# josl/kmerjs

Hardware: AMD Instinct MI355X
Metric: k-mers/sec + distinct-kmers/sec, k=16 150bp synthetic FASTQ, 1/2/4/8 GPU (higher is better)
Workload: dtype u8; 1 GPU; C2: 10000000 synthetic 150bp reads per GPU, k=16, prefix 'ATGAC'; reads_per_gpu=10000000, mode=ordered (reference Map insertion order), k=16, prefix=ATGAC, bytes_per_gpu=3170000000, pipeline=off (steps in sequence), parallelism=dp1 (one GPU; no collective), backend=none

## Files before the change

### kmerjs_amd/csrc/kmer_device.hpp

```cpp
#pragma once
#include "kmer_internal.hpp"

namespace kmerhip {

__device__ __forceinline__ uint32_t wave_incl_sum(uint32_t x) {
    x += (uint32_t)__builtin_amdgcn_update_dpp(0, (int)x, 0x111, 0xf, 0xf, true);
    x += (uint32_t)__builtin_amdgcn_update_dpp(0, (int)x, 0x112, 0xf, 0xf, true);
    x += (uint32_t)__builtin_amdgcn_update_dpp(0, (int)x, 0x114, 0xf, 0xf, true);
    x += (uint32_t)__builtin_amdgcn_update_dpp(0, (int)x, 0x118, 0xf, 0xf, true);
    x += (uint32_t)__builtin_amdgcn_update_dpp(0, (int)x, 0x142, 0xa, 0xf, false);
    x += (uint32_t)__builtin_amdgcn_update_dpp(0, (int)x, 0x143, 0xc, 0xf, false);
    return x;
}

__device__ __forceinline__ uint32_t readlane32(uint32_t v, uint32_t i) {
    return (uint32_t)__builtin_amdgcn_readlane((int)v, (int)i);
}

__device__ __forceinline__ uint64_t readlane64(uint64_t v, uint32_t i) {
    return ((uint64_t)readlane32((uint32_t)(v >> 32), i) << 32) | readlane32((uint32_t)v, i);
}

__device__ __forceinline__ void append_record(Record *recs, unsigned long long *rec_count, uint64_t rec_cap,
                                              unsigned int *err, uint64_t order, uint64_t pos, uint32_t len,
                                              uint32_t strand) {
    const unsigned long long n = atomicAdd(rec_count, 1ull);
    if (n < rec_cap) {
        Record rec;
        rec.order = order;
        rec.pos = pos;
        rec.len = len;
        rec.strand = strand;
        recs[n] = rec;
    } else {
        atomicOr(err, ERR_REC_OVERFLOW);
    }
}

__device__ __forceinline__ uint32_t nl_flags(uint32_t x) {
    uint32_t t = x ^ 0x0A0A0A0Au;
    return ~(t + 0x7F7F7F7Fu) & 0x80808080u;
}

__device__ __forceinline__ uint32_t nl_flags_below(uint32_t x, int64_t n) {
    const uint32_t z = nl_flags(x);
    return n <= 0 ? 0u : n < 4 ? (z & ((1u << (8 * n)) - 1u)) : z;
}

constexpr int NCH_MAIN = TILE / 16;
constexpr int NCH_FRONT = FH / 16;
constexpr int NCH_BACK = BH / 16;
constexpr int BUFSZ = FH + TILE + BH;

__device__ __noinline__ inline uint4 load_chunk_edge(const uint8_t *data, int64_t g, uint64_t len) {
    uint32_t w[4];
#pragma unroll 1
    for (int i = 0; i < 4; ++i) {
        uint32_t x = 0;
        for (int b = 0; b < 4; ++b) {
            const int64_t p = g + i * 4 + b;
            const uint32_t c = (p >= 0 && (uint64_t)p < len) ? data[p] : (uint32_t)'\n';
            x |= c << (8 * b);
        }
        w[i] = x;
    }
    return make_uint4(w[0], w[1], w[2], w[3]);
}

__device__ __forceinline__ uint4 load_chunk(const uint8_t *data, int64_t g, uint64_t len) {
    if (g >= 0 && (uint64_t)g + 16 <= len) return *(const uint4 *)(data + g);
    return load_chunk_edge(data, g, len);
}

struct TileRegs {
    uint4 v[4];
    uint4 vh;
    int hc;
};

__device__ __forceinline__ void load_tile(const uint8_t *data, uint64_t len, int64_t g0, TileRegs &r) {
    const int tid = threadIdx.x;
    const bool halo = tid < NCH_FRONT + NCH_BACK;
    const int hc = tid < NCH_FRONT ? tid : NCH_FRONT + NCH_MAIN + (tid - NCH_FRONT);
    r.hc = hc;
    r.vh = make_uint4(0, 0, 0, 0);
    if (g0 - FH >= 0 && (uint64_t)(g0 + TILE + BH) <= len) {
        const uint8_t *src = data + g0 + 16 * tid;
#pragma unroll
        for (int i = 0; i < 4; ++i) r.v[i] = *(const uint4 *)(src + 16 * TPB * i);
        r.vh = *(const uint4 *)(data + g0 - FH + 16 * (halo ? hc : 0));
    } else {
#pragma unroll
        for (int i = 0; i < 4; ++i) r.v[i] = load_chunk(data, g0 + (int64_t)(tid + TPB * i) * 16, len);
        if (halo) r.vh = load_chunk(data, g0 - FH + (int64_t)hc * 16, len);
    }
}

__device__ __forceinline__ uint32_t store_tile(const TileRegs &r, uint8_t *buf) {
    const int tid = threadIdx.x;
    uint32_t orall = 0;
#pragma unroll
    for (int i = 0; i < 4; ++i) {
        orall |= r.v[i].x | r.v[i].y | r.v[i].z | r.v[i].w;
        *(uint4 *)(buf + FH + (tid + TPB * i) * 16) = r.v[i];
    }
    if (tid < NCH_FRONT + NCH_BACK) *(uint4 *)(buf + r.hc * 16) = r.vh;
    return orall;
}

__device__ __forceinline__ void load_thread_words(const uint8_t *p, uint32_t (&w)[17]) {
    const uint4 *src = (const uint4 *)p;
#pragma unroll
    for (int j = 0; j < 4; ++j) {
        const uint4 x = src[j];
        w[4 * j] = x.x;
        w[4 * j + 1] = x.y;
        w[4 * j + 2] = x.z;
        w[4 * j + 3] = x.w;
    }
    w[16] = *(const uint32_t *)(p + 64);
}

}
```

### kmerjs_amd/csrc/kmer_internal.hpp

```cpp
#pragma once
#include <hip/hip_runtime.h>
#include <stdint.h>

namespace kmerhip {


constexpr int TPB = 256;
constexpr int BPT = 64;
constexpr int TILE = TPB * BPT;
constexpr int FH = 64;
constexpr int BH = 80;
constexpr int KMAX_PACKED = 32;
constexpr int KMAX_TILE = 64;
constexpr int KMAX_DENSE = 32;
constexpr uint32_t MAXREL = (1u << 23) - 1;
constexpr uint32_t PBITS_DEFAULT = 23, PBITS_LONG = 40;
constexpr uint32_t NL_SLOTS = 1024;

enum : uint32_t {
    ERR_NONASCII = 1u << 0,
    ERR_LINE_TOO_LONG = 1u << 1,
    ERR_LOOKBACK_TIMEOUT = 1u << 2,
    ERR_REC_OVERFLOW = 1u << 3,
    ERR_LINE_OVERFLOW = 1u << 4,
    ERR_OVF_OVERFLOW = 1u << 5,
    ERR_CROSS_OVERFLOW = 1u << 6,
    ERR_COUNT_OVERFLOW = 1u << 7,
    ERR_BIG_OVERFLOW = 1u << 8,
    ERR_TAB_SPLIT = 1u << 9,
    ERR_DENSE_RANK = 1u << 10,
    ERR_TAB_CAP = 1u << 11,
    ERR_BKT_CAP = 1u << 12,
    ERR_BKT_RANK = 1u << 13,
    ERR_TAB_LOOKUP = 1u << 14,
    ERR_TAB_EXTRACT = 1u << 15,
    INFO_LONGSEG = 1u << 16,
};
constexpr uint32_t CROSS_HOST_BITS = INFO_LONGSEG | ERR_OVF_OVERFLOW | ERR_REC_OVERFLOW | ERR_CROSS_OVERFLOW;

constexpr uint64_t LB_AGG = 1ull << 62;
constexpr uint64_t LB_INC = 2ull << 62;
constexpr uint64_t LB_VAL = (1ull << 62) - 1;

struct StreamPos {
    uint64_t lines;
    uint64_t unused;
    uint64_t ends_open;
    uint64_t pad;
};

struct Record {
    uint64_t order;
    uint64_t pos;
    uint32_t len;
    uint32_t strand;
};

struct SeqLine {
    uint64_t start;
    uint64_t len;
    uint64_t line_index;
};

struct HitRec {
    uint64_t code;
    uint32_t tile;
    uint32_t qm;
    uint32_t c_local;
    uint32_t lstart;
};
constexpr int HMAX = 64;

struct TileSum {
    uint64_t cnt;
    uint32_t nh;
    uint32_t nx;
    uint64_t lnl;
};

__host__ __device__ inline TileSum tile_sum_op(const TileSum &x, const TileSum &y) {
    TileSum r;
    r.cnt = x.cnt + y.cnt;
    r.nh = x.nh + y.nh;
    r.nx = x.nx + y.nx;
    r.lnl = x.lnl > y.lnl ? x.lnl : y.lnl;
    return r;
}
constexpr uint32_t TSCAN_BLOCK = 1024;
constexpr uint32_t TSCAN_INLINE_MAX = 2048;

struct ScanArgs {
    const uint8_t *data;
    uint64_t len;
    uint64_t abs_offset;
    uint32_t n_tiles, k, plen;
    uint32_t p4, r4, pmask;
    const uint8_t *PR;
    TileSum *tsum;
    HitRec *hits;
    HitRec *ovf;
    unsigned long long *ovf_count;
    uint64_t ovf_cap;
    unsigned int *err;
    uint64_t *hits_hi, *ovf_hi;
};

struct PlaneArgs {
    uint32_t kl[5], kh[5];
    uint32_t rl[5], rh[5];
    uint32_t pb;
};

struct Agg {
    uint64_t first;
    uint64_t count;
};

struct HitArgs {
    const HitRec *hits;
    const TileSum *tsum;
    const TileSum *tscan;
    const HitRec *ovf;
    const unsigned long long *ovf_count;
    uint64_t ovf_cap;
    uint32_t n_tiles, k, plen;
    uint64_t abs_offset;
    const StreamPos *pos;
    uint32_t packed;
    uint32_t pbits;
    uint64_t smask;
    uint64_t invalid_key;
    const uint64_t *hits_hi, *ovf_hi;
    uint32_t wide;
    uint64_t smask_hi;
    uint64_t *rkeyh;
    uint64_t *xkeyh, *xkeyl;
    uint64_t out_base;
    uint64_t rcap;
    uint64_t *rkey;
    uint32_t *rkey32;
    uint64_t *rord;
    uint64_t *xord, *xkey;
    uint32_t *xslot;
    uint64_t xbase, xcap;
    Record *recs;
    unsigned long long *rec_count;
    uint64_t rec_cap;
    unsigned int *err;
    const uint8_t *data;
    uint64_t len;
    uint64_t *scal;
    unsigned int *ticket;
    unsigned long long *chunk_hits, *chunk_cross, *ends_open;
    unsigned int *cross_go;
// ... 690 lines not shown
```

### kmerjs_amd/csrc/kmer_kernels.hip

```cpp
#include "kmer_device.hpp"

#include <algorithm>
#include <cstring>

namespace kmerhip {

__device__ __forceinline__ uint32_t align4(uint32_t hi, uint32_t lo, uint32_t sel) {
    return __builtin_amdgcn_alignbyte(hi, lo, sel);
}

__device__ __forceinline__ void set_info(unsigned int *err, unsigned int bit) {
    if (!(__hip_atomic_load(err, __ATOMIC_RELAXED, __HIP_MEMORY_SCOPE_AGENT) & bit)) atomicOr(err, bit);
}

__device__ __forceinline__ uint32_t not_nl_bits(uint32_t x) {
    return ((x ^ 0x0A0A0A0Au) + 0x7F7F7F7Fu) & 0x80808080u;
}

__device__ __forceinline__ uint32_t not_nl_bits_xad(uint32_t x, uint32_t k0a, uint32_t k7f) {
    uint32_t r;
    asm("v_xad_u32 %0, %1, %2, %3" : "=v"(r) : "v"(x), "v"(k0a), "s"(k7f));
    return r & 0x80808080u;
}

// ... 165 lines not shown
    const uint32_t tile = sh.tile;
    const int64_t g0 = (int64_t)tile * TILE;
    const uint64_t len = a.len;
    uint32_t w[17];
    const uint32_t total = tile_prologue(a.data, len, g0, buf, sh, w, a.err);
    const uint64_t lnl_tile = sh.lastpos >= 0 ? a.abs_offset + (uint64_t)(g0 + sh.lastpos + 1) : 0;

    if (wid == 0) {
        uint64_t lbase, lnlb;
        if (LOOKBACK) {
            if (tile == 0) {
                lbase = a.pos->lines;
                lnlb = a.abs_offset;
                if (lane == 0) {
                    lb_store(a.lb_cnt, LB_INC | (lbase + total));
                    lb_store(a.lb_lnl, LB_INC | (lnl_tile > lnlb ? lnl_tile : lnlb));
                }
            } else {
                if (lane == 0) {
                    lb_store(a.lb_cnt + tile, LB_AGG | total);
                    lb_store(a.lb_lnl + tile, LB_AGG | lnl_tile);
                }
                lbase = look_back<true>(a.lb_cnt, tile, a.err);
                lnlb = look_back<false>(a.lb_lnl, tile, a.err);
                if (lane == 0) {
                    lb_store(a.lb_cnt + tile, LB_INC | (lbase + total));
                    lb_store(a.lb_lnl + tile, LB_INC | (lnl_tile > lnlb ? lnl_tile : lnlb));
                }
            }
            if (tile == a.n_tiles - 1 && lane == 0) {
                a.pos->lines = lbase + total;
                a.pos->ends_open = (len > 0 && a.data[len - 1] != '\n') ? 1 : 0;
            }
        } else {
            lbase = a.tp_cnt[tile];
            lnlb = a.tp_lnl[tile];
        }
        if (lane == 0) {
            sh.line_base = lbase;
            sh.lnl_before = lnlb;
        }
    }
    __syncthreads();
    const uint64_t lbase = sh.line_base;
#pragma unroll 1
    for (int i = 0; i < 64; ++i) {
        const int q = 64 * tid + i;
        if ((uint64_t)(g0 + q) >= len) break;
        if (buf[FH + q - 1] != '\n') continue;
        const uint32_t c = sh.tpre[tid] + nl_before_in_thread(buf, tid, q);
        const uint64_t li = lbase + c;
        if ((li & 3) != 1) continue;
        int64_t e = g0 + q;
        while ((uint64_t)e < len && (e - g0 < TILE + BH ? buf[FH + (e - g0)] : a.data[e]) != '\n') ++e;
        const uint64_t L = (uint64_t)e - (uint64_t)(g0 + q);
        if (L > 1 && L >= a.k) {
            const unsigned long long n = atomicAdd(a.line_count, 1ull);
            if (n < a.line_cap) {
                a.lines_out[n].start = (uint64_t)(g0 + q);
                a.lines_out[n].len = L;
                a.lines_out[n].line_index = li;
            } else {
                atomicOr(a.err, ERR_LINE_OVERFLOW);
            }
        }
    }
}

constexpr int QCAP = 256;

struct alignas(16) ScanShared {
    uint16_t cpre[NCH_MAIN];
    uint32_t nlmap[NCH_MAIN / 32];
    uint32_t wsum[TPB / 64][4];
    int32_t last_chunk;
    int32_t lastpos;
    uint32_t nh;
    uint32_t nx;
    uint32_t tcnt;
    uint32_t qn;
    alignas(8) uint32_t q[QCAP];
};

__device__ __forceinline__ void put_tile_hits(const ScanArgs &a, const ScanShared &sh, uint32_t tile) {
    a.tsum[tile].nh = sh.nh;
    a.tsum[tile].nx = sh.nh > (uint32_t)HMAX ? sh.nh : sh.nx;
    if (sh.nh > (uint32_t)HMAX || (sh.nh && sh.tcnt == 0)) set_info(a.err, INFO_LONGSEG);
}

__device__ __forceinline__ int last_newline_in_chunk(const uint8_t *buf, int c, int limit = 1 << 30) {
    const uint4 x = *(const uint4 *)(buf + FH + 16 * c);
    const uint32_t xs[4] = {x.x, x.y, x.z, x.w};
    int last = -1;
#pragma unroll
    for (int j = 0; j < 4; ++j) {
        const int pos = 16 * c + 4 * j;
        const int rem = limit - pos;
        uint32_t z = nl_flags(xs[j]);
        z = rem <= 0 ? 0u : rem < 4 ? (z & ((1u << (8 * rem)) - 1u)) : z;
        last = z ? pos + ((31 - __clz(z)) >> 3) : last;
    }
    return last;
}

__host__ __device__ constexpr uint32_t byte_range_mask(int from, int to) {
    from = from < 0 ? 0 : from > 4 ? 4 : from;
    to = to < 0 ? 0 : to > 4 ? 4 : to;
    const uint32_t a = to >= 4 ? ~0u : (1u << (8 * to)) - 1u, b = from >= 4 ? ~0u : (1u << (8 * from)) - 1u;
    return a & ~b;
}

__device__ __forceinline__ uint32_t acgt_diff(uint32_t x) {
    const uint32_t c = ((x >> 1) ^ (x >> 2)) & 0x03030303u;
    return __builtin_amdgcn_perm(0u, 0x54474341u, c) ^ x;
}

__device__ __forceinline__ void line_context_chunks(const uint8_t *buf, const ScanShared &sh, int s0,
                                                    uint32_t &c_local, int &lstart) {
    const int cs = (s0 - 1) >> 4;
    const uint4 x4 = *(const uint4 *)(buf + FH + 16 * cs);
    const uint32_t xs[4] = {x4.x, x4.y, x4.z, x4.w};
    uint32_t cnt = 0;
    int last = -1;
#pragma unroll
    for (int j = 0; j < 4; ++j) {
        const int pos = 16 * cs + 4 * j;
        const int rem = s0 - pos;
        uint32_t z = nl_flags(xs[j]);
        z = rem <= 0 ? 0u : rem < 4 ? (z & ((1u << (8 * rem)) - 1u)) : z;
        cnt += __popc(z);
        last = z ? pos + ((31 - __clz(z)) >> 3) : last;
    }
    c_local = (uint32_t)sh.cpre[cs] + cnt;
    if (last >= 0) {
        lstart = last + 1;
    } else if (c_local > 0) {
        const int cc = cs - 1;
        int wi = cc >> 5;
        uint32_t m = sh.nlmap[wi] & (0xFFFFFFFFu >> (31 - (cc & 31)));
        while (m == 0) m = sh.nlmap[--wi];
        lstart = last_newline_in_chunk(buf, 32 * wi + 31 - __clz(m)) + 1;
    }
}

__device__ __forceinline__ uint32_t chunk_nl_mask(uint4 x) {
    const uint32_t k0a = 0x0A0A0A0Au, k7f = 0x7F7F7F7Fu;
    const uint32_t lo = __builtin_amdgcn_udot4(not_nl_bits_xad(x.y, k0a, k7f), 0x80402010u,
                            __builtin_amdgcn_udot4(not_nl_bits_xad(x.x, k0a, k7f), 0x08040201u, 0u, false), false);
    const uint32_t hi = __builtin_amdgcn_udot4(not_nl_bits_xad(x.w, k0a, k7f), 0x80402010u,
                            __builtin_amdgcn_udot4(not_nl_bits_xad(x.z, k0a, k7f), 0x08040201u, 0u, false), false);
    return ~((lo >> 7) | (hi << 1)) & 0xFFFFu;
}

__device__ __forceinline__ void line_context_regions(const uint8_t *buf, const ScanShared &sh, int s0, bool want,
                                                     uint32_t &c_local, int &lstart) {
    const int cs = (s0 > 0 ? s0 - 1 : 0) >> 4;
    const int rg = cs >> 2, wi = rg >> 5;
    const uint4 x4 = *(const uint4 *)(buf + FH + 16 * cs);
    const uint2 c2 = *(const uint2 *)(sh.cpre + 4 * rg);
    const uint32_t mhi = sh.nlmap[wi], mlo = sh.nlmap[wi > 0 ? wi - 1 : 0];
    const uint32_t cnt = __popc(__builtin_amdgcn_ubfe(chunk_nl_mask(x4), 0u, (uint32_t)(s0 - 16 * cs)));
    const uint32_t ccs = (uint32_t)((((uint64_t)c2.y << 32) | c2.x) >> (16 * (cs & 3))) & 0xFFFFu;
    const uint32_t cl = ccs + cnt;
    const bool has = want && cl > 0;
    int R = rg;
    if (has && cnt == 0 && ccs == (c2.x & 0xFFFFu)) {
        const uint64_t m = (((uint64_t)mhi << 32) | (wi > 0 ? mlo : 0u)) & ((1ull << (32 + (rg & 31))) - 1ull);
        R = 32 * (wi - 1) + 63 - (int)__clzll((long long)m);
        if (m == 0) {
            int w = wi - 1;
            uint32_t mm;
            do mm = sh.nlmap[--w]; while (mm == 0);
            R = 32 * w + 31 - __clz(mm);
        }
    }
    const uint2 d2 = *(const uint2 *)(sh.cpre + 4 * R);
    const uint32_t nxt = sh.cpre[min(4 * R + 4, NCH_MAIN - 1)];
    const uint32_t d[4] = {d2.x & 0xFFFFu, d2.x >> 16, d2.y & 0xFFFFu, d2.y >> 16};
    const int jl = R == rg ? cs - 4 * rg : 4;
    const int jc = (jl > 3 && d[3] < nxt) ? 3 : (jl > 2 && d[2] < d[3]) ? 2 : (jl > 1 && d[1] < d[2]) ? 1 : 0;
    const int c = cnt ? cs : 4 * R + jc;
    const uint4 y4 = *(const uint4 *)(buf + FH + 16 * c);
    const uint32_t ym = __builtin_amdgcn_ubfe(chunk_nl_mask(y4), 0u, (uint32_t)min(s0 - 16 * c, 16));
    const int last = 16 * c + 31 - __clz(ym);
    c_local = want ? cl : 0u;
    lstart = has ? last + 1 : -1;
}

template <bool THREAD_MAP, bool WIDE, uint32_t K = 0, uint32_t PLEN = 0>
__device__ __forceinline__ void emit_hit(const ScanArgs &a, const uint8_t *buf, ScanShared &sh, uint32_t tile,
                                         uint32_t e, uint32_t pb = 0, const uint32_t *pw = nullptr) {
    static_assert((K == 0) == (PLEN == 0) && PLEN <= 5 && PLEN <= K && K <= (WIDE ? KMAX_TILE : KMAX_PACKED),
                  "fixed k / prefix length: both or neither, prefix fully plane-tested");
    const uint32_t k = K ? K : a.k, plen = K ? PLEN : a.plen;
    const uint32_t strand = e & 1u;
    const int q = (int)(e >> 1);
    const int s0 = strand ? q + (int)plen - (int)k : q;
    uint32_t exo_bits = 0, nl_bits = 0;
    uint32_t pfx_bits = 0;
    uint64_t code = 0;
    const int sfx0 = strand ? 0 : (int)plen, sfx1 = strand ? (int)(k - plen) : (int)k;
#pragma unroll 4
    for (uint32_t b = 0; b < k; b += 4) {
        const uint32_t x = lds_word(buf, s0 + (int)b);
        const uint32_t nb = k - b >= 4 ? 4u : k - b;
        const uint32_t mk = nb == 4 ? 0xFFFFFFFFu : ((1u << (8 * nb)) - 1u);
        const uint32_t c = ((x >> 1) ^ (x >> 2)) & 0x03030303u;
        const uint32_t expect = __builtin_amdgcn_perm(0u, 0x54474341u, c);
        if (THREAD_MAP && K) {
            const uint32_t pf = byte_range_mask(0 - (int)b, (int)PLEN - (int)b),
                           pr = byte_range_mask((int)K - (int)PLEN - (int)b, (int)K - (int)b);
            const uint32_t pm = strand ? pr : pf;
            pfx_bits |= (expect ^ x) & mk & pm;
            exo_bits |= (expect ^ x) & mk & ~pm;
        } else {
            const uint32_t mx = THREAD_MAP ? mk : mk & byte_range_mask(sfx0 - (int)b, sfx1 - (int)b);
            exo_bits |= (expect ^ x) & mx;
        }
        nl_bits |= nl_flags(x) & mk;
        const uint32_t pk = __builtin_amdgcn_udot4(c, 0x01041040u, 0u, false);
        code = (code << (2 * nb)) | (pk >> (2 * (4 - nb)));
    }
    if (THREAD_MAP && !K) {
        pfx_bits = (acgt_diff(lds_word(buf, q)) & (pb >= 4 ? 0xFFFFFFFFu : ((1u << (8 * pb)) - 1u))) |
                   (acgt_diff(lds_word(buf, q + 4)) & (pb > 4 ? 0xFFu : 0u));
        for (uint32_t b = 4; b < plen && plen > 5; b += 4) {
            const uint32_t n = plen - b;
            const uint32_t mk = (n >= 4 ? 0xFFFFFFFFu : ((1u << (8 * n)) - 1u)) & (b == 4 ? 0xFFFFFF00u : 0xFFFFFFFFu);
            pfx_bits |= (lds_word(buf, q + (int)b) ^ pw[(strand ? KMAX_TILE / 4 : 0) + b / 4]) & mk;
        }
    }
    const bool exotic = exo_bits != 0, hasnl = nl_bits != 0;
    uint64_t chi = 0;
    if (WIDE) {
        for (uint32_t b = 0; b < k - 32; b += 4) {
            const uint32_t x = lds_word(buf, s0 + (int)b);
            const uint32_t nb = k - 32 - b >= 4 ? 4u : k - 32 - b;
            const uint32_t c = ((x >> 1) ^ (x >> 2)) & 0x03030303u;
            const uint32_t pk = __builtin_amdgcn_udot4(c, 0x01041040u, 0u, false);
            chi = (chi << (2 * nb)) | (pk >> (2 * (4 - nb)));
        }
    }
    const bool valid = pfx_bits == 0 && !hasnl &&
                       !(k == 1 && buf[FH + s0 - 1] == '\n' && buf[FH + s0 + 1] == '\n');
    uint32_t c_local = 0;
    int lstart = -1;
    if (THREAD_MAP) line_context_regions(buf, sh, s0, valid && s0 > 0, c_local, lstart);
    else if (valid && s0 > 0) line_context_chunks(buf, sh, s0, c_local, lstart);
    const bool cross = valid && (lstart < 0 || c_local == sh.tcnt);
    const unsigned long long vm = __ballot(valid), xm = __ballot(cross), act = __ballot(1);
    const int lane = threadIdx.x & 63, leader = __ffsll((long long)act) - 1;
    uint32_t base = 0;
    if (lane == leader) {
        if (vm) base = atomicAdd(&sh.nh, (uint32_t)__popcll(vm));
        if (xm) atomicAdd(&sh.nx, (uint32_t)__popcll(xm));
    }
    base = (uint32_t)__shfl((int)base, leader);
    if (!valid) return;
    const uint32_t slot = base + (uint32_t)__popcll(vm & ((1ull << lane) - 1ull));
    HitRec r;
    r.code = code;
    r.tile = tile;
    r.qm = (uint32_t)q | (strand << 14) | ((exotic ? 1u : 0u) << 15) | ((lstart >= 0 ? 1u : 0u) << 16) | (slot << 17);
    r.c_local = c_local;
    r.lstart = lstart >= 0 ? (uint32_t)lstart : 0u;
    if (slot < HMAX) {
        a.hits[(uint64_t)tile * HMAX + slot] = r;
        if (WIDE) a.hits_hi[(uint64_t)tile * HMAX + slot] = chi;
    } else {
        const unsigned long long o = atomicAdd(a.ovf_count, 1ull);
        if (o < a.ovf_cap) {
            a.ovf[o] = r;
            if (WIDE) a.ovf_hi[o] = chi;
        } else {
            atomicOr(a.err, ERR_OVF_OVERFLOW);
        }
    }
}

template <bool WIDE>
__device__ __forceinline__ void scan_word(const ScanArgs &a, const uint8_t *buf, ScanShared &sh, uint32_t tile,
                                          const uint32_t *pw, uint32_t q0) {
    const uint32_t plen = a.plen, P4 = a.p4, R4 = a.r4, PM = a.pmask;
    const uint32_t lo = *(const uint32_t *)(buf + FH + q0);
    const uint32_t hi = *(const uint32_t *)(buf + FH + q0 + 4);
    uint32_t bits = 0;
#pragma unroll
    for (uint32_t jj = 0; jj < 4; ++jj) {
        const uint32_t win = align4(hi, lo, jj);
        bits |= (((win ^ P4) & PM) == 0 ? 1u : 0u) << (2 * jj);
        bits |= (((win ^ R4) & PM) == 0 ? 1u : 0u) << (2 * jj + 1);
    }
    while (bits) {
        const uint32_t bit = __ffs(bits) - 1;
        bits &= bits - 1;
        const uint32_t strand = bit & 1u;
        const int q = (int)q0 + (int)(bit >> 1);
        bool ok = true;
#pragma unroll 1
        for (uint32_t b = 4; b < plen && ok; b += 4) {
            const uint32_t n = plen - b;
            const uint32_t mk = n >= 4 ? 0xFFFFFFFFu : ((1u << (8 * n)) - 1u);
            ok = ((lds_word(buf, q + (int)b) ^ pw[(strand ? KMAX_TILE / 4 : 0) + b / 4]) & mk) == 0;
        }
        if (ok) emit_hit<false, WIDE>(a, buf, sh, tile, ((uint32_t)q << 1) | strand);
    }
}

template <bool FULL4, bool WIDE>
__global__ __launch_bounds__(TPB) void scan_tile_kernel(ScanArgs a) {
    __shared__ __attribute__((aligned(16))) uint8_t buf[BUFSZ];
    __shared__ ScanShared sh;
    __shared__ __attribute__((aligned(16))) uint8_t s_pr[2 * KMAX_TILE];
    const int tid = threadIdx.x, lane = tid & 63, wid = tid >> 6;
    const uint64_t len = a.len;
    const uint32_t tile = blockIdx.x;
    const int64_t g0 = (int64_t)tile * TILE;
    {
        uint8_t prb = 0;
        if (tid < 2 * KMAX_TILE) prb = a.PR[tid];
        TileRegs r;
        load_tile(a.data, len, g0, r);
        if (tid == 0) {
            sh.last_chunk = -1;
            sh.nh = 0;
            sh.nx = 0;
            sh.qn = 0;
        }
        const uint32_t orall = store_tile(r, buf);
        if (tid < 2 * KMAX_TILE) s_pr[tid] = prb;
        if (orall & 0x80808080u) atomicOr(a.err, ERR_NONASCII);
    }
// ... 63 lines not shown
            }
        }
        const uint64_t excl = incl - packed;
        uint32_t base = 0;
#pragma unroll
        for (int i = 0; i < 4; ++i) {
            sh.cpre[tid + TPB * i] = (uint16_t)(base + col_off[i] + ((excl >> (16 * i)) & 0xFFFFu));
            base += col_total[i];
        }
        if (tid == 0) {
            a.tsum[tile].cnt = base;
            sh.tcnt = base;
        }
    }
    if (tid == 0) {
        const int lc = sh.last_chunk;
        const int64_t lim = (int64_t)len - g0;
        const int lp = lc >= 0 ? last_newline_in_chunk(buf, lc, lim < TILE ? (int)lim : TILE) : -1;
        sh.lastpos = lp;
        a.tsum[tile].lnl = lp >= 0 ? a.abs_offset + (uint64_t)(g0 + lp + 1) : 0;
    }
    const uint32_t k = a.k, plen = a.plen;
    if (plen > k) cand = 0;
    const uint32_t *pw = (const uint32_t *)s_pr;

    __syncthreads();
    {
        const uint32_t nc = __popc(cand);
        const uint32_t incl_c = wave_incl_sum(nc);
        const uint32_t wtotal = (uint32_t)__builtin_amdgcn_readlane((int)incl_c, 63);
        uint32_t pos = 0;
        if (wtotal) {
            uint32_t base = 0;
            if (lane == 0) base = atomicAdd(&sh.qn, wtotal);
            pos = (uint32_t)__builtin_amdgcn_readfirstlane((int)__shfl((int)base, 0)) + incl_c - nc;
        }
        while (cand) {
            const int bitc = __ffs(cand) - 1;
            cand &= cand - 1;
            const uint32_t q0 = 16u * (uint32_t)(tid + TPB * (bitc >> 2)) + 4u * (uint32_t)(bitc & 3);
            if (pos < QCAP) sh.q[pos] = q0;
            else scan_word<WIDE>(a, buf, sh, tile, pw, q0);
            ++pos;
        }
    }
    __syncthreads();
    const uint32_t nq = min(sh.qn, (uint32_t)QCAP);
    for (uint32_t h = tid; h < nq; h += TPB) scan_word<WIDE>(a, buf, sh, tile, pw, sh.q[h]);
    if (nq > 64 || sh.qn > QCAP) {
        __syncthreads();
        if (tid == 0) put_tile_hits(a, sh, tile);
    } else if (tid == 0) {
        put_tile_hits(a, sh, tile);
    }
}


__device__ __forceinline__ uint32_t plane_match(uint32_t L0, uint32_t H0, uint32_t L1, uint32_t H1,
                                                const uint32_t *kl, const uint32_t *kh, uint32_t pb,
                                                const uint32_t *SL, const uint32_t *SH) {
    uint32_t acc = (L0 ^ kl[0]) & (H0 ^ kh[0]);
#pragma unroll
    for (uint32_t i = 1; i < 5; ++i) {
        if (i < pb) acc = acc & (SL[i] ^ kl[i]) & (SH[i] ^ kh[i]);
    }
    return acc;
}

__host__ __device__ constexpr uint32_t plane_masks_const(const char *p, const char *r) {
    uint32_t m = 0;
    for (int i = 0; i < 5; ++i) {
        const uint32_t cp = (((uint32_t)p[i] >> 1) & 1u) | ((((uint32_t)p[i] >> 2) & 1u) << 1);
        const uint32_t cr = (((uint32_t)r[i] >> 1) & 1u) | ((((uint32_t)r[i] >> 2) & 1u) << 1);
        m |= ((cp & 1u) ? 0u : 1u) << (4 * i);
        m |= ((cp & 2u) ? 0u : 1u) << (4 * i + 1);
        m |= ((cr & 1u) ? 0u : 1u) << (4 * i + 2);
        m |= ((cr & 2u) ? 0u : 1u) << (4 * i + 3);
    }
    return m;
}
constexpr uint32_t PM_ATGAC = plane_masks_const("ATGAC", "GTCAT");

template <bool FULL5, bool WIDE, uint32_t PM = 0, uint32_t K = 0, uint32_t PLEN = 0>
__global__ __launch_bounds__(TPB) void scan_planes_kernel(ScanArgs a, PlaneArgs pa) {
    __shared__ __attribute__((aligned(16))) uint8_t buf[BUFSZ];
    __shared__ ScanShared sh;
    __shared__ __attribute__((aligned(16))) uint8_t s_pr[2 * KMAX_TILE];
    const int tid = threadIdx.x, lane = tid & 63, wid = tid >> 6;
    const uint64_t len = a.len;
    const uint32_t tile = blockIdx.x;
    const int64_t g0 = (int64_t)tile * TILE;
    {
        uint8_t prb = 0;
        if (K == 0 && tid < 2 * KMAX_TILE) prb = a.PR[tid];
        TileRegs r;
        load_tile(a.data, len, g0, r);
        if (tid == 0) {
            sh.last_chunk = -1;
            sh.nh = 0;
            sh.nx = 0;
            sh.qn = 0;
        }
        const uint32_t orall = store_tile(r, buf);
        if (K == 0 && tid < 2 * KMAX_TILE) s_pr[tid] = prb;
        if (orall & 0x80808080u) atomicOr(a.err, ERR_NONASCII);
    }
    __syncthreads();

    uint32_t w[17];
    load_thread_words(buf + FH + 64 * tid, w);
    const bool tail_tile = (uint64_t)(g0 + TILE) > len;
    const uint32_t k0a = 0x0A0A0A0Au, k7f = 0x7F7F7F7Fu;
    uint32_t ccnt[4];
#pragma unroll
    for (int j = 0; j < 4; ++j) {
        uint32_t cnt = 0;
        if (!tail_tile) {
#pragma unroll
            for (int i = 0; i < 4; ++i) cnt += __popc(not_nl_bits_xad(w[4 * j + i], k0a, k7f));
            cnt = 16u - cnt;
        } else {
            const int64_t gc = g0 + 64 * tid + 16 * j;
#pragma unroll
            for (int i = 0; i < 4; ++i) cnt += __popc(nl_flags_below(w[4 * j + i], (int64_t)len - (gc + 4 * i)));
        }
        ccnt[j] = cnt;
    }
    const uint32_t ttot = ccnt[0] + ccnt[1] + ccnt[2] + ccnt[3];
    {
        const unsigned long long m = __ballot(ttot != 0);
        if (lane == 0) {
            sh.nlmap[2 * wid] = (uint32_t)m;
            sh.nlmap[2 * wid + 1] = (uint32_t)(m >> 32);
            if (m) atomicMax(&sh.last_chunk, 64 * wid + 63 - (int)__clzll((long long)m));
        }
    }
    const uint32_t incl = wave_incl_sum(ttot);
    if (lane == 63) sh.wsum[wid][0] = incl;

    const uint32_t W0 = 0x08040201u;
    uint32_t L[3], H[3];
#pragma unroll
    for (int h = 0; h < 2; ++h) {
        uint32_t gl[4], gh[4];
#pragma unroll
        for (int p = 0; p < 4; ++p) {
            const uint32_t x0 = w[8 * h + 2 * p], x1 = w[8 * h + 2 * p + 1];
            uint32_t y;
            asm("v_bfi_b32 %0, %1, %2, %3" : "=v"(y) : "s"(0x0F0F0F0Fu), "v"(x0), "v"(x1 << 4));
            gl[p] = __builtin_amdgcn_udot4(y & 0x22222222u, W0, 0u, false);
            gh[p] = __builtin_amdgcn_udot4(y & 0x44444444u, W0, 0u, false);
        }
        L[h] = (gl[0] >> 1) | (gl[1] << 7) | (gl[2] << 15) | (gl[3] << 23);
        H[h] = (gh[0] >> 2) | (gh[1] << 6) | (gh[2] << 14) | (gh[3] << 22);
    }
    {
        const uint32_t x = w[16];
        L[2] = __builtin_amdgcn_udot4(x & 0x02020202u, W0, 0u, false) >> 1;
        H[2] = __builtin_amdgcn_udot4(x & 0x04040404u, W0, 0u, false) >> 2;
    }
    uint32_t mf[2], mr[2];
    const uint32_t pb = FULL5 ? 5u : pa.pb;
    uint32_t kl[5], kh[5], rl[5], rh[5];
#pragma unroll
    for (int i = 0; i < 5; ++i) {
        if constexpr (PM != 0) {
            kl[i] = ((PM >> (4 * i)) & 1u) ? ~0u : 0u;
            kh[i] = ((PM >> (4 * i + 1)) & 1u) ? ~0u : 0u;
            rl[i] = ((PM >> (4 * i + 2)) & 1u) ? ~0u : 0u;
            rh[i] = ((PM >> (4 * i + 3)) & 1u) ? ~0u : 0u;
        } else {
            kl[i] = pa.kl[i];
            kh[i] = pa.kh[i];
            rl[i] = pa.rl[i];
            rh[i] = pa.rh[i];
        }
    }
#pragma unroll
    for (int h = 0; h < 2; ++h) {
        uint32_t SL[5], SH[5];
        SL[0] = L[h];
        SH[0] = H[h];
#pragma unroll
        for (uint32_t i = 1; i < 5; ++i) {
            SL[i] = __builtin_amdgcn_alignbit(L[h + 1], L[h], i);
            SH[i] = __builtin_amdgcn_alignbit(H[h + 1], H[h], i);
        }
        mf[h] = plane_match(L[h], H[h], L[h + 1], H[h + 1], kl, kh, pb, SL, SH);
        mr[h] = plane_match(L[h], H[h], L[h + 1], H[h + 1], rl, rh, pb, SL, SH);
    }
    if (!K && a.k < a.plen) mf[0] = mf[1] = mr[0] = mr[1] = 0;

    __syncthreads();
    {
        uint32_t pre = incl - ttot, tot = 0;
#pragma unroll
        for (int ww = 0; ww < TPB / 64; ++ww) {
            pre += ww < wid ? sh.wsum[ww][0] : 0u;
            tot += sh.wsum[ww][0];
        }
#pragma unroll
        for (int j = 0; j < 4; ++j) {
            sh.cpre[4 * tid + j] = (uint16_t)pre;
            pre += ccnt[j];
        }
        if (tid == 0) {
            a.tsum[tile].cnt = tot;
            sh.tcnt = tot;
        }
    }
    __syncthreads();
    if (tid == 0) {
        const int lt = sh.last_chunk;
        int lp = -1;
        if (lt >= 0) {
            int c = 4 * lt + 3;
            while ((c == NCH_MAIN - 1 ? sh.tcnt : (uint32_t)sh.cpre[c + 1]) == sh.cpre[c]) --c;
            const int64_t lim = (int64_t)len - g0;
            lp = last_newline_in_chunk(buf, c, lim < TILE ? (int)lim : TILE);
        }
        sh.lastpos = lp;
        a.tsum[tile].lnl = lp >= 0 ? a.abs_offset + (uint64_t)(g0 + lp + 1) : 0;
    }

    const uint32_t *pw = (const uint32_t *)s_pr;
    uint2 *qe = (uint2 *)sh.q;
    constexpr uint32_t QE = QCAP / 2;
    static_assert(QE == 128 && QCAP == 256, "a round: one entry per thread of waves 0 and 1, 128 queue words each");
    const uint32_t mm[4] = {mf[0], mf[1], mr[0], mr[1]};
    uint32_t qpos[4] = {0, 0, 0, 0};
    {
        unsigned long long bl[4];
        uint32_t tot = 0;
#pragma unroll
        for (int hs = 0; hs < 4; ++hs) {
            bl[hs] = __ballot(mm[hs] != 0);
            tot += (uint32_t)__popcll(bl[hs]);
        }
        if (tot) {
            uint32_t base = 0;
            if (lane == 0) base = atomicAdd(&sh.qn, tot);
            base = (uint32_t)__builtin_amdgcn_readfirstlane((int)base);
#pragma unroll
            for (int hs = 0; hs < 4; ++hs) {
                qpos[hs] = base + __builtin_amdgcn_mbcnt_hi((uint32_t)(bl[hs] >> 32),
                                                            __builtin_amdgcn_mbcnt_lo((uint32_t)bl[hs], 0u));
                base += (uint32_t)__popcll(bl[hs]);
            }
        }
    }
    auto enqueue = [&](uint32_t done) {
#pragma unroll
        for (int hs = 0; hs < 4; ++hs) {
            const uint32_t e0 = ((64u * (uint32_t)tid + 32u * (uint32_t)(hs & 1)) << 1) | (uint32_t)(hs >> 1);
            if (mm[hs] && qpos[hs] - done < QE) qe[qpos[hs] - done] = make_uint2(e0, mm[hs]);
        }
    };
    enqueue(0);
    __syncthreads();
    const uint32_t total = sh.qn;
    if (total <= 64 && wid != 0) return;
    for (uint32_t done = 0;;) {
        const uint32_t left = total - done;
        uint2 en = make_uint2(0u, 0u);
        if ((uint32_t)tid < min(left, QE)) en = qe[tid];
        const uint32_t nc = __popc(en.y), incl = wave_incl_sum(nc);
        const uint32_t wtot = readlane32(incl, 63);
        uint32_t *flat = sh.q + 128 * (wid & 1);
        for (uint32_t cb = 0; cb < wtot; cb += 64) {
            uint32_t m = en.y, p = incl - nc - cb;
            while (m) {
                const uint32_t bit = __ffs(m) - 1;
                m &= m - 1;
                if (p < 64) flat[p] = en.x + (bit << 1);
                ++p;
            }
            if ((uint32_t)lane < min(wtot - cb, 64u))
                emit_hit<true, WIDE, K, PLEN>(a, buf, sh, tile, flat[lane], pb, pw);
        }
        if (left <= QE) break;
        __syncthreads();
        done += QE;
        enqueue(done);
        __syncthreads();
    }
    if (total > 64) __syncthreads();
    if (tid == 0) put_tile_hits(a, sh, tile);
}

__device__ __forceinline__ uint64_t resolve_hit(const HitArgs &a, uint64_t pos_lines, const HitRec &r,
                                                uint64_t code_hi, const TileSum &tb, uint64_t *order_out,
                                                uint32_t *lk, bool *lvalid_out, uint64_t *key_hi) {
    const uint32_t t = r.tile;
    const uint32_t strand = (r.qm >> 14) & 1u;
    const bool exotic = (r.qm >> 15) & 1u;
    const bool lvalid = (r.qm >> 16) & 1u;
    const int q = (int)(r.qm & 0x3FFFu);
    const int s0 = strand ? q + (int)a.plen - (int)a.k : q;
    const uint64_t tile_abs = a.abs_offset + (uint64_t)t * TILE;
    const uint64_t li = pos_lines + tb.cnt + r.c_local;
    const uint64_t lstart = lvalid ? tile_abs + r.lstart : tb.lnl;
    const uint64_t sabs = tile_abs + (uint64_t)(int64_t)s0;
    uint64_t rel = sabs - lstart;
    const bool seq = (li & 3) == 1;
    const uint64_t maxrel = (1ull << a.pbits) - 1ull;
    if (rel > maxrel) {
        if (seq) atomicOr(a.err, ERR_LINE_TOO_LONG);
        rel = maxrel;
    }
    if (li >> (63 - a.pbits)) atomicOr(a.err, ERR_LINE_TOO_LONG);
    const uint64_t order = (li << (a.pbits + 1)) | ((uint64_t)strand << a.pbits) | (strand ? maxrel - rel : rel);
    *order_out = order;
    const uint32_t sp = (uint32_t)(s0 + 64);
    *lk = (r.c_local << 17) | (strand << 16) | (strand ? 0xFFFFu - sp : sp);
    *lvalid_out = lvalid;
    uint64_t key = a.invalid_key;
    *key_hi = a.wide ? a.invalid_key : 0;
    if (a.wide) key = 0;
    if (seq) {
        if (a.packed && !exotic) {
            if (a.k > 32) {
                uint64_t h = code_hi, l = r.code;
                if (strand) revcomp_code128(code_hi, r.code, a.k, &h, &l);
                key = l & a.smask;
                *key_hi = h & a.smask_hi;
            } else {
                key = (strand ? revcomp_code(r.code, a.k) : r.code) & a.smask;
            }
        } else {
            append_record(a.recs, a.rec_count, a.rec_cap, a.err, order, (uint64_t)t * TILE + (uint64_t)(int64_t)s0, a.k,
                          strand);
        }
    }
    return key;
}

__device__ __forceinline__ void place_hit(const HitArgs &a, uint64_t slot, bool cross, uint64_t xi, uint64_t key,
                                          uint64_t key_hi, uint64_t order) {
    if (!cross) {
        if (slot >= a.rcap) {
            atomicOr(a.err, ERR_OVF_OVERFLOW);
            return;
        }
        if (a.rkey32) a.rkey32[slot] = (uint32_t)key;
        else a.rkey[slot] = key;
        if (a.wide) a.rkeyh[slot] = key_hi;
        a.rord[slot] = order;
    } else if (xi < a.xcap) {
        a.xord[xi] = order;
        a.xslot[xi] = (uint32_t)slot;
        if (a.wide) {
            a.xkey[xi] = xi;
            a.xkeyl[xi] = key;
            a.xkeyh[xi] = key_hi;
        } else {
            a.xkey[xi] = key;
        }
    } else {
        atomicOr(a.err, ERR_CROSS_OVERFLOW);
    }
}
// ... 2359 lines not shown
```

Measured before the change: 3487 billion k-mers/s.

## Carry per-hit line context in queue and drop barrier-heavy prefix pass in plane scan

The plane-scan kernel no longer builds a shared per-chunk newline prefix table or runs the serial last-newline search behind two extra block barriers. Each thread computes a 64-bit newline mask, a wave prefix count and a wave max of its last-newline position, and stores this context next to its queued hits. Emitters then derive the line start and local count from that mask with popcount/clz instead of walking shared tables. The change also adds nontemporal loads for the main tile and an 8-waves-per-EU occupancy hint, at the cost of a larger shared struct (a 16-byte context per queue entry) and extra packing logic on the queue entries.

After: 3795 billion k-mers/s (median of 6 runs). 1.09x the previous value.

```diff
diff --git a/kmerjs_amd/csrc/kmer_device.hpp b/kmerjs_amd/csrc/kmer_device.hpp
--- a/kmerjs_amd/csrc/kmer_device.hpp
+++ b/kmerjs_amd/csrc/kmer_device.hpp
@@ -10,6 +10,16 @@
     x += (uint32_t)__builtin_amdgcn_update_dpp(0, (int)x, 0x118, 0xf, 0xf, true);
     x += (uint32_t)__builtin_amdgcn_update_dpp(0, (int)x, 0x142, 0xa, 0xf, false);
     x += (uint32_t)__builtin_amdgcn_update_dpp(0, (int)x, 0x143, 0xc, 0xf, false);
+    return x;
+}
+
+__device__ __forceinline__ uint32_t wave_incl_max(uint32_t x) {
+    x = max(x, (uint32_t)__builtin_amdgcn_update_dpp(0, (int)x, 0x111, 0xf, 0xf, true));
+    x = max(x, (uint32_t)__builtin_amdgcn_update_dpp(0, (int)x, 0x112, 0xf, 0xf, true));
+    x = max(x, (uint32_t)__builtin_amdgcn_update_dpp(0, (int)x, 0x114, 0xf, 0xf, true));
+    x = max(x, (uint32_t)__builtin_amdgcn_update_dpp(0, (int)x, 0x118, 0xf, 0xf, true));
+    x = max(x, (uint32_t)__builtin_amdgcn_update_dpp(0, (int)x, 0x142, 0xa, 0xf, false));
+    x = max(x, (uint32_t)__builtin_amdgcn_update_dpp(0, (int)x, 0x143, 0xc, 0xf, false));
     return x;
 }
 
@@ -78,6 +88,7 @@
     int hc;
 };
 
+template <bool NT = false>
 __device__ __forceinline__ void load_tile(const uint8_t *data, uint64_t len, int64_t g0, TileRegs &r) {
     const int tid = threadIdx.x;
     const bool halo = tid < NCH_FRONT + NCH_BACK;
@@ -87,7 +98,15 @@
     if (g0 - FH >= 0 && (uint64_t)(g0 + TILE + BH) <= len) {
         const uint8_t *src = data + g0 + 16 * tid;
 #pragma unroll
-        for (int i = 0; i < 4; ++i) r.v[i] = *(const uint4 *)(src + 16 * TPB * i);
+        for (int i = 0; i < 4; ++i) {
+            if constexpr (NT) {
+                typedef uint32_t u32x4 __attribute__((ext_vector_type(4)));
+                const u32x4 t = __builtin_nontemporal_load((const u32x4 *)(src + 16 * TPB * i));
+                r.v[i] = make_uint4(t.x, t.y, t.z, t.w);
+            } else {
+                r.v[i] = *(const uint4 *)(src + 16 * TPB * i);
+            }
+        }
         r.vh = *(const uint4 *)(data + g0 - FH + 16 * (halo ? hc : 0));
     } else {
 #pragma unroll
diff --git a/kmerjs_amd/csrc/kmer_internal.hpp b/kmerjs_amd/csrc/kmer_internal.hpp
--- a/kmerjs_amd/csrc/kmer_internal.hpp
+++ b/kmerjs_amd/csrc/kmer_internal.hpp
@@ -70,6 +70,16 @@
     uint32_t lstart;
 };
 constexpr int HMAX = 64;
+
+__host__ __device__ inline void region_line_context(uint32_t pre, int32_t prevnl, uint64_t mask, uint32_t qrel,
+                                                    int32_t base, uint32_t *c_local, int32_t *lstart) {
+    const uint64_t below = mask & ((1ull << qrel) - 1ull);
+    const uint32_t lo = (uint32_t)below, hi = (uint32_t)(below >> 32);
+    *c_local = pre + (uint32_t)__builtin_popcount(lo) + (uint32_t)__builtin_popcount(hi);
+    const int32_t own = hi ? 64 - __builtin_clz(hi) : 32 - __builtin_clz(lo | 1u);
+    const int32_t ls = below ? base + own : prevnl + 1;
+    *lstart = ls > 0 ? ls : -1;
+}
 
 struct TileSum {
     uint64_t cnt;
diff --git a/kmerjs_amd/csrc/kmer_kernels.hip b/kmerjs_amd/csrc/kmer_kernels.hip
--- a/kmerjs_amd/csrc/kmer_kernels.hip
+++ b/kmerjs_amd/csrc/kmer_kernels.hip
@@ -271,7 +271,21 @@
     alignas(8) uint32_t q[QCAP];
 };
 
-__device__ __forceinline__ void put_tile_hits(const ScanArgs &a, const ScanShared &sh, uint32_t tile) {
+constexpr uint32_t QE = QCAP / 2;
+struct alignas(16) PlaneShared {
+    uint32_t wsum[TPB / 64];
+    uint32_t wmax[TPB / 64];
+    uint32_t nh;
+    uint32_t nx;
+    uint32_t tcnt;
+    uint32_t qn;
+    uint2 q[QE];
+    uint4 qc[QE];
+    uint32_t flat[2][64];
+};
+
+template <class SH>
+__device__ __forceinline__ void put_tile_hits(const ScanArgs &a, const SH &sh, uint32_t tile) {
     a.tsum[tile].nh = sh.nh;
     a.tsum[tile].nx = sh.nh > (uint32_t)HMAX ? sh.nh : sh.nx;
     if (sh.nh > (uint32_t)HMAX || (sh.nh && sh.tcnt == 0)) set_info(a.err, INFO_LONGSEG);
@@ -332,53 +346,10 @@
     }
 }
 
-__device__ __forceinline__ uint32_t chunk_nl_mask(uint4 x) {
-    const uint32_t k0a = 0x0A0A0A0Au, k7f = 0x7F7F7F7Fu;
-    const uint32_t lo = __builtin_amdgcn_udot4(not_nl_bits_xad(x.y, k0a, k7f), 0x80402010u,
-                            __builtin_amdgcn_udot4(not_nl_bits_xad(x.x, k0a, k7f), 0x08040201u, 0u, false), false);
-    const uint32_t hi = __builtin_amdgcn_udot4(not_nl_bits_xad(x.w, k0a, k7f), 0x80402010u,
-                            __builtin_amdgcn_udot4(not_nl_bits_xad(x.z, k0a, k7f), 0x08040201u, 0u, false), false);
-    return ~((lo >> 7) | (hi << 1)) & 0xFFFFu;
-}
-
-__device__ __forceinline__ void line_context_regions(const uint8_t *buf, const ScanShared &sh, int s0, bool want,
-                                                     uint32_t &c_local, int &lstart) {
-    const int cs = (s0 > 0 ? s0 - 1 : 0) >> 4;
-    const int rg = cs >> 2, wi = rg >> 5;
-    const uint4 x4 = *(const uint4 *)(buf + FH + 16 * cs);
-    const uint2 c2 = *(const uint2 *)(sh.cpre + 4 * rg);
-    const uint32_t mhi = sh.nlmap[wi], mlo = sh.nlmap[wi > 0 ? wi - 1 : 0];
-    const uint32_t cnt = __popc(__builtin_amdgcn_ubfe(chunk_nl_mask(x4), 0u, (uint32_t)(s0 - 16 * cs)));
-    const uint32_t ccs = (uint32_t)((((uint64_t)c2.y << 32) | c2.x) >> (16 * (cs & 3))) & 0xFFFFu;
-    const uint32_t cl = ccs + cnt;
-    const bool has = want && cl > 0;
-    int R = rg;
-    if (has && cnt == 0 && ccs == (c2.x & 0xFFFFu)) {
-        const uint64_t m = (((uint64_t)mhi << 32) | (wi > 0 ? mlo : 0u)) & ((1ull << (32 + (rg & 31))) - 1ull);
-        R = 32 * (wi - 1) + 63 - (int)__clzll((long long)m);
-        if (m == 0) {
-            int w = wi - 1;
-            uint32_t mm;
-            do mm = sh.nlmap[--w]; while (mm == 0);
-            R = 32 * w + 31 - __clz(mm);
-        }
-    }
-    const uint2 d2 = *(const uint2 *)(sh.cpre + 4 * R);
-    const uint32_t nxt = sh.cpre[min(4 * R + 4, NCH_MAIN - 1)];
-    const uint32_t d[4] = {d2.x & 0xFFFFu, d2.x >> 16, d2.y & 0xFFFFu, d2.y >> 16};
-    const int jl = R == rg ? cs - 4 * rg : 4;
-    const int jc = (jl > 3 && d[3] < nxt) ? 3 : (jl > 2 && d[2] < d[3]) ? 2 : (jl > 1 && d[1] < d[2]) ? 1 : 0;
-    const int c = cnt ? cs : 4 * R + jc;
-    const uint4 y4 = *(const uint4 *)(buf + FH + 16 * c);
-    const uint32_t ym = __builtin_amdgcn_ubfe(chunk_nl_mask(y4), 0u, (uint32_t)min(s0 - 16 * c, 16));
-    const int last = 16 * c + 31 - __clz(ym);
-    c_local = want ? cl : 0u;
-    lstart = has ? last + 1 : -1;
-}
-
-template <bool THREAD_MAP, bool WIDE, uint32_t K = 0, uint32_t PLEN = 0>
-__device__ __forceinline__ void emit_hit(const ScanArgs &a, const uint8_t *buf, ScanShared &sh, uint32_t tile,
-                                         uint32_t e, uint32_t pb = 0, const uint32_t *pw = nullptr) {
+template <bool THREAD_MAP, bool WIDE, uint32_t K = 0, uint32_t PLEN = 0, class SH>
+__device__ __forceinline__ void emit_hit(const ScanArgs &a, const uint8_t *buf, SH &sh, uint32_t tile,
+                                         uint32_t e, uint32_t pb = 0, const uint32_t *pw = nullptr,
+                                         uint4 lc = make_uint4(0u, 0u, 0u, 0u), uint32_t tcnt = 0) {
     static_assert((K == 0) == (PLEN == 0) && PLEN <= 5 && PLEN <= K && K <= (WIDE ? KMAX_TILE : KMAX_PACKED),
                   "fixed k / prefix length: both or neither, prefix fully plane-tested");
     const uint32_t k = K ? K : a.k, plen = K ? PLEN : a.plen;
@@ -434,9 +405,14 @@
                        !(k == 1 && buf[FH + s0 - 1] == '\n' && buf[FH + s0 + 1] == '\n');
     uint32_t c_local = 0;
     int lstart = -1;
-    if (THREAD_MAP) line_context_regions(buf, sh, s0, valid && s0 > 0, c_local, lstart);
-    else if (valid && s0 > 0) line_context_chunks(buf, sh, s0, c_local, lstart);
-    const bool cross = valid && (lstart < 0 || c_local == sh.tcnt);
+    if constexpr (THREAD_MAP) {
+        region_line_context(lc.x, (int)lc.w - 1, ((uint64_t)lc.z << 32) | lc.y, (uint32_t)q & 63u, q & ~63, &c_local,
+                            &lstart);
+    } else {
+        if (valid && s0 > 0) line_context_chunks(buf, sh, s0, c_local, lstart);
+        tcnt = sh.tcnt;
+    }
+    const bool cross = valid && (lstart < 0 || c_local == tcnt);
     const unsigned long long vm = __ballot(valid), xm = __ballot(cross), act = __ballot(1);
     const int lane = threadIdx.x & 63, leader = __ffsll((long long)act) - 1;
     uint32_t base = 0;
@@ -666,9 +642,9 @@
 constexpr uint32_t PM_ATGAC = plane_masks_const("ATGAC", "GTCAT");
 
 template <bool FULL5, bool WIDE, uint32_t PM = 0, uint32_t K = 0, uint32_t PLEN = 0>
-__global__ __launch_bounds__(TPB) void scan_planes_kernel(ScanArgs a, PlaneArgs pa) {
+__global__ __launch_bounds__(TPB) __attribute__((amdgpu_waves_per_eu(8))) void scan_planes_kernel(ScanArgs a, PlaneArgs pa) {
     __shared__ __attribute__((aligned(16))) uint8_t buf[BUFSZ];
-    __shared__ ScanShared sh;
+    __shared__ PlaneShared sh;
     __shared__ __attribute__((aligned(16))) uint8_t s_pr[2 * KMAX_TILE];
     const int tid = threadIdx.x, lane = tid & 63, wid = tid >> 6;
     const uint64_t len = a.len;
@@ -678,9 +654,8 @@
         uint8_t prb = 0;
         if (K == 0 && tid < 2 * KMAX_TILE) prb = a.PR[tid];
         TileRegs r;
-        load_tile(a.data, len, g0, r);
+        load_tile<true>(a.data, len, g0, r);
         if (tid == 0) {
-            sh.last_chunk = -1;
             sh.nh = 0;
             sh.nx = 0;
             sh.qn = 0;
@@ -695,32 +670,32 @@
     load_thread_words(buf + FH + 64 * tid, w);
     const bool tail_tile = (uint64_t)(g0 + TILE) > len;
     const uint32_t k0a = 0x0A0A0A0Au, k7f = 0x7F7F7F7Fu;
-    uint32_t ccnt[4];
-#pragma unroll
-    for (int j = 0; j < 4; ++j) {
-        uint32_t cnt = 0;
-        if (!tail_tile) {
-#pragma unroll
-            for (int i = 0; i < 4; ++i) cnt += __popc(not_nl_bits_xad(w[4 * j + i], k0a, k7f));
-            cnt = 16u - cnt;
-        } else {
-            const int64_t gc = g0 + 64 * tid + 16 * j;
-#pragma unroll
-            for (int i = 0; i < 4; ++i) cnt += __popc(nl_flags_below(w[4 * j + i], (int64_t)len - (gc + 4 * i)));
-        }
-        ccnt[j] = cnt;
-    }
-    const uint32_t ttot = ccnt[0] + ccnt[1] + ccnt[2] + ccnt[3];
-    {
-        const unsigned long long m = __ballot(ttot != 0);
-        if (lane == 0) {
-            sh.nlmap[2 * wid] = (uint32_t)m;
-            sh.nlmap[2 * wid + 1] = (uint32_t)(m >> 32);
-            if (m) atomicMax(&sh.last_chunk, 64 * wid + 63 - (int)__clzll((long long)m));
-        }
-    }
+    uint32_t nm[2];
+#pragma unroll
+    for (int h = 0; h < 2; ++h) {
+        uint32_t d[4];
+#pragma unroll
+        for (int p = 0; p < 4; ++p)
+            d[p] = __builtin_amdgcn_udot4(not_nl_bits_xad(w[8 * h + 2 * p + 1], k0a, k7f), 0x80402010u,
+                       __builtin_amdgcn_udot4(not_nl_bits_xad(w[8 * h + 2 * p], k0a, k7f), 0x08040201u, 0u, false), false);
+        nm[h] = ~((d[0] >> 7) | (d[1] << 1) | (d[2] << 9) | (d[3] << 17));
+    }
+    if (tail_tile) {
+        const int64_t left = (int64_t)len - (g0 + 64 * tid);
+        const uint64_t keep = left >= 64 ? ~0ull : left <= 0 ? 0ull : (1ull << left) - 1ull;
+        nm[0] &= (uint32_t)keep;
+        nm[1] &= (uint32_t)(keep >> 32);
+    }
+    const uint32_t ttot = __popc(nm[0]) + __popc(nm[1]);
+    const uint32_t mylast = nm[1] ? 64u * (uint32_t)tid + 64u - (uint32_t)__clz(nm[1])
+                                  : nm[0] ? 64u * (uint32_t)tid + 32u - (uint32_t)__clz(nm[0]) : 0u;
     const uint32_t incl = wave_incl_sum(ttot);
-    if (lane == 63) sh.wsum[wid][0] = incl;
+    const uint32_t inclmax = wave_incl_max(mylast);
+    if (lane == 63) {
+        sh.wsum[wid] = incl;
+        sh.wmax[wid] = inclmax;
+    }
+    uint32_t prev1 = (uint32_t)__builtin_amdgcn_update_dpp(0, (int)inclmax, 0x138, 0xf, 0xf, true);
 
     const uint32_t W0 = 0x08040201u;
     uint32_t L[3], H[3];
@@ -775,42 +750,10 @@
     }
     if (!K && a.k < a.plen) mf[0] = mf[1] = mr[0] = mr[1] = 0;
 
-    __syncthreads();
-    {
-        uint32_t pre = incl - ttot, tot = 0;
-#pragma unroll
-        for (int ww = 0; ww < TPB / 64; ++ww) {
-            pre += ww < wid ? sh.wsum[ww][0] : 0u;
-            tot += sh.wsum[ww][0];
-        }
-#pragma unroll
-        for (int j = 0; j < 4; ++j) {
-            sh.cpre[4 * tid + j] = (uint16_t)pre;
-            pre += ccnt[j];
-        }
-        if (tid == 0) {
-            a.tsum[tile].cnt = tot;
-            sh.tcnt = tot;
-        }
-    }
-    __syncthreads();
-    if (tid == 0) {
-        const int lt = sh.last_chunk;
-        int lp = -1;
-        if (lt >= 0) {
-            int c = 4 * lt + 3;
-            while ((c == NCH_MAIN - 1 ? sh.tcnt : (uint32_t)sh.cpre[c + 1]) == sh.cpre[c]) --c;
-            const int64_t lim = (int64_t)len - g0;
-            lp = last_newline_in_chunk(buf, c, lim < TILE ? (int)lim : TILE);
-        }
-        sh.lastpos = lp;
-        a.tsum[tile].lnl = lp >= 0 ? a.abs_offset + (uint64_t)(g0 + lp + 1) : 0;
-    }
-
     const uint32_t *pw = (const uint32_t *)s_pr;
-    uint2 *qe = (uint2 *)sh.q;
-    constexpr uint32_t QE = QCAP / 2;
-    static_assert(QE == 128 && QCAP == 256, "a round: one entry per thread of waves 0 and 1, 128 queue words each");
+    uint2 *qe = sh.q;
+    static_assert(QE == 128, "a round: one entry per thread of waves 0 and 1");
+    const uint4 myctx = make_uint4((incl - ttot) | (prev1 << 16), nm[0], nm[1], 0u);
     const uint32_t mm[4] = {mf[0], mf[1], mr[0], mr[1]};
     uint32_t qpos[4] = {0, 0, 0, 0};
     {
@@ -837,30 +780,58 @@
 #pragma unroll
         for (int hs = 0; hs < 4; ++hs) {
             const uint32_t e0 = ((64u * (uint32_t)tid + 32u * (uint32_t)(hs & 1)) << 1) | (uint32_t)(hs >> 1);
-            if (mm[hs] && qpos[hs] - done < QE) qe[qpos[hs] - done] = make_uint2(e0, mm[hs]);
+            if (mm[hs] && qpos[hs] - done < QE) {
+                qe[qpos[hs] - done] = make_uint2(e0, mm[hs]);
+                sh.qc[qpos[hs] - done] = myctx;
+            }
         }
     };
     enqueue(0);
     __syncthreads();
     const uint32_t total = sh.qn;
     if (total <= 64 && wid != 0) return;
+    uint32_t wpre[TPB / 64], wprev[TPB / 64], tcnt = 0, tlast = 0;
+    {
+        const uint4 ws = *(const uint4 *)sh.wsum, wm = *(const uint4 *)sh.wmax;
+        const uint32_t s[4] = {ws.x, ws.y, ws.z, ws.w}, m[4] = {wm.x, wm.y, wm.z, wm.w};
+#pragma unroll
+        for (int ww = 0; ww < TPB / 64; ++ww) {
+            wpre[ww] = tcnt;
+            wprev[ww] = tlast;
+            tcnt += (uint32_t)__builtin_amdgcn_readfirstlane((int)s[ww]);
+            tlast = max(tlast, (uint32_t)__builtin_amdgcn_readfirstlane((int)m[ww]));
+        }
+    }
+    if (tid == 0) {
+        a.tsum[tile].cnt = tcnt;
+        a.tsum[tile].lnl = tlast ? a.abs_offset + (uint64_t)(g0 + tlast) : 0;
+        sh.tcnt = tcnt;
+    }
     for (uint32_t done = 0;;) {
         const uint32_t left = total - done;
         uint2 en = make_uint2(0u, 0u);
         if ((uint32_t)tid < min(left, QE)) en = qe[tid];
         const uint32_t nc = __popc(en.y), incl = wave_incl_sum(nc);
         const uint32_t wtot = readlane32(incl, 63);
-        uint32_t *flat = sh.q + 128 * (wid & 1);
+        uint32_t *flat = sh.flat[wid & 1];
         for (uint32_t cb = 0; cb < wtot; cb += 64) {
             uint32_t m = en.y, p = incl - nc - cb;
             while (m) {
                 const uint32_t bit = __ffs(m) - 1;
                 m &= m - 1;
-                if (p < 64) flat[p] = en.x + (bit << 1);
+                if (p < 64) flat[p] = (en.x + (bit << 1)) | ((uint32_t)tid << 16);
                 ++p;
             }
-            if ((uint32_t)lane < min(wtot - cb, 64u))
-                emit_hit<true, WIDE, K, PLEN>(a, buf, sh, tile, flat[lane], pb, pw);
+            if ((uint32_t)lane < min(wtot - cb, 64u)) {
+                const uint32_t f = flat[lane], ow = (f >> 13) & 3u;
+                uint4 lc = sh.qc[f >> 16];
+                const uint32_t wp = ow == 0 ? wpre[0] : ow == 1 ? wpre[1] : ow == 2 ? wpre[2] : wpre[3];
+                const uint32_t wl = ow == 0 ? wprev[0] : ow == 1 ? wprev[1] : ow == 2 ? wprev[2] : wprev[3];
+                const uint32_t prv = lc.x >> 16;
+                lc.x = (lc.x & 0xFFFFu) + wp;
+                lc.w = prv ? prv : wl;
+                emit_hit<true, WIDE, K, PLEN>(a, buf, sh, tile, f & 0xFFFFu, pb, pw, lc, tcnt);
+            }
         }
         if (left <= QE) break;
         __syncthreads();
```
